# syzhang092218-source/dgppo

Measured on AMD Instinct MI355X. Metric: env-steps/sec whole node, LidarSpread n=8 4096 envs, 1/2/4/8 GPUs, higher is better.
Workload: dtype f32

## Files before the change

### dgppo_amd/csrc/nn_graph.hip

```cpp
#include "common.h"

struct Topo {
  int n, ng, gs, os, per, lidar, spread;
  int S, Ns;
};

static Topo make_topo(const dgppo_env_cfg& c) {
  Topo t;
  t.n = c.n_agents; t.ng = c.n_goals; t.gs = cfg_goal_slots(c); t.os = cfg_obs_slots(c);
  t.lidar = cfg_is_lidar(c) ? 1 : 0; t.spread = cfg_is_spread(c) ? 1 : 0;
  t.per = t.os;
  t.S = t.n + t.gs + t.os;
  t.Ns = t.n + t.ng + cfg_obs_nodes(c);
  return t;
}

__device__ inline int sender_node(const Topo& t, int i, int s) {
  if (s < t.n) return s;
  if (s < t.n + t.gs) return t.spread ? t.n + (s - t.n) : t.n + i;
  const int m = s - t.n - t.gs;
  return t.lidar ? t.n + t.ng + i * t.per + m : t.n + t.ng + m;
}
__device__ inline int slot_of(const Topo& t, int nd, int i) {
  if (nd < t.n) return nd;
// ... 165 lines not shown
  const float* qt;
  const float* Xa;
  const float* Xo;
  const float* efeat;
  const float* emask;
  float* zcat;
  float* attn;
  const float* dzcat;
  float* dqt;
  float* dXa;
  float* dXo;
  int relu_xo;
  int G;
  const float* Xo_raw; const float* Wo; const float* bo; int ldwo;
  float* dwo_slab;
};

__global__ void __launch_bounds__(256) attn_fwd_valu_kernel(AttnArgs a) {
  extern __shared__ float sm[];
  const Topo& t = a.t;
  const int g = blockIdx.x, tid = threadIdx.x, nt = blockDim.x;
  const int n = t.n, S = t.S, Ns = t.Ns, F = a.F, H = a.H, Fl = F + 1;
  float* s_x = sm;
  float* s_q = s_x + Ns * Fl;
  float* s_e = s_q + n * H * Fl;
  float* s_m = s_e + n * S * 4;
  float* s_a = s_m + n * S;
  for (int idx = tid; idx < Ns * F; idx += nt) {
    const int nd = idx / F, f = idx - nd * F;
    s_x[nd * Fl + f] = (nd < n) ? a.Xa[((size_t)g * n + nd) * F + f] : a.Xo[((size_t)g * (Ns - n) + (nd - n)) * F + f];
// ... 354 lines not shown
  return __int_as_float(__builtin_amdgcn_update_dpp(0, __float_as_int(v), CTRL, 0xf, 0xf, false));
}
__device__ inline float grp8_sum(float v) {
  v += dpp_f<0xB1>(v);
  v += dpp_f<0x4E>(v);
  v += dpp_f<0x141>(v);
  return v;
}
__device__ inline float grp8_max(float v) {
  v = fmaxf(v, dpp_f<0xB1>(v));
  v = fmaxf(v, dpp_f<0x4E>(v));
  v = fmaxf(v, dpp_f<0x141>(v));
  return v;
}

template <int H, int NPA, int SJ>
__global__ void __launch_bounds__(256) attn_fwd_slot8_kernel(AttnArgs a) {
  constexpr int F = 8, Wd = F + 4;
  const Topo& t = a.t;
  const int lane = threadIdx.x & 63, wave = threadIdx.x >> 6, sub = lane & 7, grp = lane >> 3;
  const int g = __builtin_amdgcn_readfirstlane(blockIdx.x * 4 + wave);
  if (g >= a.G) return;
  const int n = t.n, S = t.S, Ns = t.Ns, Kp = a.Kp, kc = F + H * Wd;
  const float* Xa = a.Xa + (size_t)g * n * F;
  const float* Xo = a.Xo + (size_t)g * (Ns - n) * F - (size_t)n * F;
  const float* qt = a.qt + (size_t)g * n * H * F;
  const float* ef = a.efeat + (size_t)g * n * S * 4;
  const float* mk = a.emask + (size_t)g * n * S;
  float* zc = a.zcat + (size_t)g * n * Kp;
  float* at = a.attn + (size_t)g * n * S * H;
  for (int idx = lane; idx < n * 2; idx += 64)
    *reinterpret_cast<float4*>(zc + (idx >> 1) * Kp + 4 * (idx & 1)) = reinterpret_cast<const float4*>(Xa)[idx];
  for (int i = lane; i < n; i += 64)
    for (int c = kc; c < Kp; ++c) zc[i * Kp + c] = (c == kc) ? ones_col(a.t, mk + i * S) : 0.0f;
#pragma unroll
  for (int p = 0; p < NPA; ++p) {
    const int ia = grp + 8 * p;
    const bool live = ia < n;
    const int i = live ? ia : n - 1;
    float4 q[H][2], x[SJ][2], e[SJ];
    float m[SJ];
#pragma unroll
    for (int h = 0; h < H; ++h) {
      const float4* qp = reinterpret_cast<const float4*>(qt + (i * H + h) * F);
      q[h][0] = qp[0]; q[h][1] = qp[1];
    }
#pragma unroll
    for (int j = 0; j < SJ; ++j) {
      int sl = sub + 8 * j;
      sl = sl < S ? sl : S - 1;
      const int nd = sender_node(t, i, sl);
      const float4* xp = reinterpret_cast<const float4*>((nd < n ? Xa : Xo) + (size_t)nd * F);
      x[j][0] = xp[0]; x[j][1] = xp[1];
      e[j] = reinterpret_cast<const float4*>(ef)[i * S + sl];
      m[j] = mk[i * S + sl];
    }
    float av[SJ][H];
#pragma unroll
    for (int h = 0; h < H; ++h) {
      float mx = -INFINITY;
#pragma unroll
      for (int j = 0; j < SJ; ++j) {
        const bool ok = live && (sub + 8 * j) < S && m[j] != 0.0f;
        float acc = q[h][0].x * x[j][0].x;
        acc = fmaf(q[h][0].y, x[j][0].y, acc); acc = fmaf(q[h][0].z, x[j][0].z, acc); acc = fmaf(q[h][0].w, x[j][0].w, acc);
        acc = fmaf(q[h][1].x, x[j][1].x, acc); acc = fmaf(q[h][1].y, x[j][1].y, acc);
        acc = fmaf(q[h][1].z, x[j][1].z, acc); acc = fmaf(q[h][1].w, x[j][1].w, acc);
        av[j][h] = ok ? acc : -INFINITY;
        mx = fmaxf(mx, av[j][h]);
      }
      mx = grp8_max(mx);
      float den = 0.0f;
#pragma unroll
      for (int j = 0; j < SJ; ++j) {
        const float ev = (av[j][h] == -INFINITY) ? 0.0f : __expf(av[j][h] - mx);
        av[j][h] = ev;
        den += ev;
      }
      den = grp8_sum(den);
      const float inv = (den > 0.0f) ? 1.0f / den : 0.0f;
#pragma unroll
      for (int j = 0; j < SJ; ++j) av[j][h] *= inv;
    }
#pragma unroll
    for (int j = 0; j < SJ; ++j) {
      const int sl = sub + 8 * j;
      if (live && sl < S) {
#pragma unroll
        for (int h = 0; h < H; ++h) if (a.attn != nullptr) at[(i * S + sl) * H + h] = av[j][h];
      }
    }
#pragma unroll
    for (int h = 0; h < H; ++h) {
      float z[Wd];
#pragma unroll
      for (int c = 0; c < Wd; ++c) z[c] = 0.0f;
#pragma unroll
      for (int j = 0; j < SJ; ++j) {
        const float w = av[j][h];
        if (w != 0.0f) {
          z[0] = fmaf(w, x[j][0].x, z[0]); z[1] = fmaf(w, x[j][0].y, z[1]); z[2] = fmaf(w, x[j][0].z, z[2]); z[3] = fmaf(w, x[j][0].w, z[3]);
          z[4] = fmaf(w, x[j][1].x, z[4]); z[5] = fmaf(w, x[j][1].y, z[5]); z[6] = fmaf(w, x[j][1].z, z[6]); z[7] = fmaf(w, x[j][1].w, z[7]);
          z[8] = fmaf(w, e[j].x, z[8]); z[9] = fmaf(w, e[j].y, z[9]); z[10] = fmaf(w, e[j].z, z[10]); z[11] = fmaf(w, e[j].w, z[11]);
        }
      }
#pragma unroll
      for (int c = 0; c < Wd; ++c) z[c] = grp8_sum(z[c]);
      if (live && sub == h) {
        float4* o = reinterpret_cast<float4*>(zc + i * Kp + F + h * Wd);
        o[0] = make_float4(z[0], z[1], z[2], z[3]);
        o[1] = make_float4(z[4], z[5], z[6], z[7]);
        o[2] = make_float4(z[8], z[9], z[10], z[11]);
      }
    }
  }
}

template <int H, int NPA, int SJ>
__global__ void __launch_bounds__(256) attn_bwd_slot8_kernel(AttnArgs a) {
  constexpr int F = 8, Wd = F + 4;
  const Topo& t = a.t;
  const int lane = threadIdx.x & 63, wave = threadIdx.x >> 6, sub = lane & 7, grp = lane >> 3;
  const int g = __builtin_amdgcn_readfirstlane(blockIdx.x * 4 + wave);
  if (g >= a.G) return;
  const int n = t.n, S = t.S, Ns = t.Ns, Kp = a.Kp;
  const float* Xa = a.Xa + (size_t)g * n * F;
  const float* Xo = a.Xo + (size_t)g * (Ns - n) * F - (size_t)n * F;
// ... 57 lines not shown
          o[0] = fmaf(dl, x[j][0].x, o[0]); o[1] = fmaf(dl, x[j][0].y, o[1]); o[2] = fmaf(dl, x[j][0].z, o[2]); o[3] = fmaf(dl, x[j][0].w, o[3]);
          o[4] = fmaf(dl, x[j][1].x, o[4]); o[5] = fmaf(dl, x[j][1].y, o[5]); o[6] = fmaf(dl, x[j][1].z, o[6]); o[7] = fmaf(dl, x[j][1].w, o[7]);
        }
      }
#pragma unroll
      for (int c = 0; c < F; ++c) o[c] = grp8_sum(o[c]);
      if (live && sub == h) {
        float4* op = reinterpret_cast<float4*>(dq + (i * H + h) * F);
        op[0] = make_float4(o[0], o[1], o[2], o[3]);
        op[1] = make_float4(o[4], o[5], o[6], o[7]);
      }
    }
  }
}

template <int H, int NPA>
static bool launch_attn_slot8_sj(const AttnArgs& a, int SJ, int grid, hipStream_t s, bool bwd) {
#define DGPPO_SJ(J)                                                                                              \
  case J:                                                                                                        \
    if (bwd) hipLaunchKernelGGL((attn_bwd_slot8_kernel<H, NPA, J>), dim3(grid), dim3(256), 0, s, a);             \
    else hipLaunchKernelGGL((attn_fwd_slot8_kernel<H, NPA, J>), dim3(grid), dim3(256), 0, s, a);                 \
    return true;
  switch (SJ) {
    DGPPO_SJ(1) DGPPO_SJ(2) DGPPO_SJ(3) DGPPO_SJ(4) DGPPO_SJ(5) DGPPO_SJ(6) DGPPO_SJ(7) DGPPO_SJ(8)
    default: return false;
  }
#undef DGPPO_SJ
}
static bool attn_slot8_shape(const Topo& t, int F, int H) { return F == 8 && H == 3 && t.n <= 32 && t.S <= 64; }
static bool launch_attn_slot8(const AttnArgs& a, hipStream_t s, bool bwd) {
  if (!attn_slot8_shape(a.t, a.F, a.H)) return false;
  const int grid = (a.G + 3) / 4, NPA = (a.t.n + 7) / 8, SJ = (a.t.S + 7) / 8;
  switch (NPA) {
    case 1: return launch_attn_slot8_sj<3, 1>(a, SJ, grid, s, bwd);
    case 2: return launch_attn_slot8_sj<3, 2>(a, SJ, grid, s, bwd);
    case 3: return launch_attn_slot8_sj<3, 3>(a, SJ, grid, s, bwd);
    case 4: return launch_attn_slot8_sj<3, 4>(a, SJ, grid, s, bwd);
    default: return false;
  }
}

#define ABD_XL 36
#define ABD_DZL 40
typedef float4 abd_f4;
__device__ inline f32x4g mfma4(float a_, float b_, f32x4g c_) { return __builtin_amdgcn_mfma_f32_4x4x1f32(a_, b_, c_, 0, 0, 0); }
__device__ inline const float* f4e(const float4& v) { return reinterpret_cast<const float*>(&v); }
__device__ inline float4 ld4_if(bool ok, const float4* p) {
  float4 v = make_float4(0.f, 0.f, 0.f, 0.f);
  if (ok) v = *p;
  return v;
}

// ... 1112 lines not shown
                                  float* attn, int32_t G, void* stream) {
  AttnArgs a{};
  int32_t rc = attn_check(cfg, F, H, Kp, G, a);
  if (rc) return rc;
  if (G == 0) return 0;
  DGPPO_REQUIRE(qt && Xa && efeat && emask && zcat, "attn_fwd: NULL operand");
  DGPPO_REQUIRE(a.t.Ns == a.t.n || Xo, "attn_fwd: Xo is NULL");
  a.qt = qt; a.Xa = Xa; a.Xo = Xo; a.efeat = efeat; a.emask = emask; a.zcat = zcat; a.attn = attn;
  const Topo& t = a.t;
  const hipStream_t s = (hipStream_t)stream;
  const size_t smem = sizeof(float) * ((size_t)t.Ns * (F + 1) + (size_t)t.n * H * (F + 1) + (size_t)t.n * t.S * 5 +
                                       (size_t)t.n * t.S * H);
  DGPPO_REQUIRE(smem <= 64 * 1024, "attn_fwd: graph too large for LDS (%zu B)", smem);
  bool launched = true;
  switch (attn_family(t, F, H, Kp, false, false)) {
    case AttnFamily::SLOT8: launched = launch_attn_slot8(a, s, false); break;
    case AttnFamily::BD: launched = launch_attn_bd(a, s, false); break;
    case AttnFamily::MFMA:
      hipLaunchKernelGGL(attn_fwd_kernel, dim3(G), dim3(256), attn_mfma_smem(attn_dims(t, F, H), false), s, a);
      break;
    case AttnFamily::VALU: hipLaunchKernelGGL(attn_fwd_valu_kernel, dim3(G), dim3(256), smem, s, a); break;
  }
  DGPPO_REQUIRE(launched, "attn_fwd: dispatch failed");
  DGPPO_LAUNCH_CHECK();
  return 0;
}

extern "C" int32_t dgppo_attn_bwd(const dgppo_env_cfg* cfg, int32_t F, int32_t H, int32_t Kp, const float* dzcat,
                                  const float* attn, const float* qt, const float* Xa, const float* Xo,
                                  const float* efeat, float* dqt, float* dXa, float* dXo, int32_t relu_xo, int32_t G,
                                  void* stream) {
  AttnArgs a{};
  int32_t rc = attn_check(cfg, F, H, Kp, G, a);
  if (rc) return rc;
  if (G == 0) return 0;
  DGPPO_REQUIRE(dzcat && attn && qt && Xa && efeat && dqt, "attn_bwd: NULL operand");
  DGPPO_REQUIRE(a.t.Ns == a.t.n || Xo, "attn_bwd: Xo is NULL");
  DGPPO_REQUIRE(!(dXo && !dXa), "attn_bwd: dXo needs dXa");
  a.dzcat = dzcat; a.attn = (float*)attn; a.qt = qt; a.Xa = Xa; a.Xo = Xo; a.efeat = efeat; a.dqt = dqt; a.dXa = dXa; a.dXo = dXo;
  const Topo& t = a.t;
  const hipStream_t s = (hipStream_t)stream;
  const size_t smem = sizeof(float) * ((size_t)t.Ns * (F + 1) + (size_t)t.n * H * (F + 1) + (size_t)t.n * t.S * 4 +
                                       2 * (size_t)t.n * t.S * H + (size_t)t.n * H * (F + 5));
  DGPPO_REQUIRE(smem <= 64 * 1024, "attn_bwd: graph too large for LDS (%zu B)", smem);
  const AttnFamily fam = attn_family(t, F, H, Kp, true, dXa != nullptr);
  a.relu_xo = (relu_xo && dXo && fam == AttnFamily::BD) ? 1 : 0;
  bool launched = true;
  switch (fam) {
    case AttnFamily::SLOT8: launched = launch_attn_slot8(a, s, true); break;
    case AttnFamily::BD: launched = launch_attn_bd(a, s, true); break;
    case AttnFamily::MFMA:
      hipLaunchKernelGGL(attn_bwd_kernel, dim3(G), dim3(256), attn_mfma_smem(attn_dims(t, F, H), true), s, a);
      break;
    case AttnFamily::VALU: hipLaunchKernelGGL(attn_bwd_valu_kernel, dim3(G), dim3(256), smem, s, a); break;
  }
  DGPPO_REQUIRE(launched, "attn_bwd: dispatch failed");
  DGPPO_LAUNCH_CHECK();
  if (relu_xo && dXo && !a.relu_xo)
    return dgppo_relu_bwd(dXo, Xo, (int64_t)G * (t.Ns - t.n) * F, stream);
  return 0;
}

static bool attn_xo_ok(const Topo& t, int F, int H, int Kp) {
  return t.Ns > t.n && attn_family(t, F, H, Kp, true, true) == AttnFamily::BD;
}
extern "C" int32_t dgppo_attn_xo_supported(const dgppo_env_cfg* cfg, int32_t F, int32_t H, int32_t Kp) {
  AttnArgs a{};
  if (attn_check(cfg, F, H, Kp, 0, a)) return 0;
  return attn_xo_ok(a.t, F, H, Kp) ? 1 : 0;
}
extern "C" int32_t dgppo_attn_fwd_xo(const dgppo_env_cfg* cfg, int32_t F, int32_t H, int32_t Kp, const float* qt, const float* Xa,
                                     const float* Xo_raw, const float* Wo, int32_t ldwo, const float* bo, const float* efeat,
                                     const float* emask, float* zcat, float* attn, int32_t G, void* stream) {
  AttnArgs a{};
// ... 79 lines not shown
```

### dgppo_amd/nets.py

```python
from __future__ import annotations

import math
from typing import Dict, List, Optional, Tuple

import numpy as np
import torch

from . import _native as N
from . import ops_nn as K

H_HEADS = 3
MSG_DIM = 32
OUT_DIM = 64
HID = 64


def _ceil4(x):
    return (x + 3) // 4 * 4


class Layout:
    def __init__(self):
        self.entries: Dict[str, Tuple[int, Tuple[int, ...]]] = {}
        self.size = 0
# ... 162 lines not shown
        for l, (f, fp, d, kp) in enumerate(self.dims):
            q = lambda nm: self.p(f"gnn{l}.{nm}")
            K.gnn_prep(q("Wq"), q("bq"), q("Wk"), q("Wv"), q("bv"), q("We"), q("Wu"), self.pp(f"gnn{l}.Mcat"),
                       self.pp(f"gnn{l}.cvec"), self.pp(f"gnn{l}.Wout"), f, fp, d, H_HEADS, kp)

    def _xo_fusable(self, l: int) -> bool:
        if l != 0 or self.gnn_layers != 2:
            return False
        key = "_xo_ok"
        if not hasattr(self, key):
            f1, fp1, d1, kp1 = self.dims[1]
            setattr(self, key, self.dims[0][1] == 8 and self.dims[0][2] == 32 and fp1 == 32 and
                    K.attn_xo_supported(self.cfg, fp1, H_HEADS, kp1))
        return getattr(self, key)

    def zero_grads(self):
        self.grads.zero_()

    def forward(self, feats: GraphFeats, n_seq: int, T: int, h0: Optional[torch.Tensor], tag: str = "f",
                hs_out: Optional[torch.Tensor] = None, train: bool = True):
        cfg, G, A = self.cfg, feats.G, self.arena
        n = cfg.n_agents
        R = G * n
        Ro = G * feats.n_other
        act = {"feats": feats, "G": G, "n_seq": n_seq, "T": T}
        Xa, Xo = feats.Xa, feats.Xo
        xo_fused = None
        for l, (f, fp, d, kp) in enumerate(self.dims):
            qt = A.get(f"{tag}.qt{l}", R, H_HEADS * fp)
            K.dense_fwd(Xa, self.pp(f"gnn{l}.Mcat"), self.pp(f"gnn{l}.cvec"), qt)
            zcat = A.get(f"{tag}.zcat{l}", R, kp)
            attn = A.get(f"{tag}.attn{l}", R, cfg.fan_in, H_HEADS) if train else None
            if xo_fused is not None:
                K.attn_fwd_xo(cfg, fp, H_HEADS, kp, qt, Xa, xo_fused[0], xo_fused[1], xo_fused[2], feats.efeat, feats.emask, zcat, attn, G)
            else:
                K.attn_fwd(cfg, fp, H_HEADS, kp, qt, Xa, Xo if Ro > 0 else None, feats.efeat, feats.emask, zcat, attn, G)
            act[f"xo_fused{l}"] = xo_fused
            xo_fused = None
            Xa_n = A.get(f"{tag}.Xa{l + 1}", R, d)
            K.dense_fwd(zcat, self.pp(f"gnn{l}.Wout"), self.p(f"gnn{l}.bu"), Xa_n, act=1)
            act[f"Xa{l}"], act[f"Xo{l}"], act[f"qt{l}"], act[f"zcat{l}"], act[f"attn{l}"] = Xa, Xo, qt, zcat, attn
            if l < self.gnn_layers - 1 and Ro > 0:
                if self._xo_fusable(l):
                    xo_fused = (Xo, self.pp(f"gnn{l}.Wout")[:fp], self.p(f"gnn{l}.bu"))
                    Xo = None
                else:
                    Xo_n = A.get(f"{tag}.Xo{l + 1}", Ro, d)
                    K.dense_fwd(Xo, self.pp(f"gnn{l}.Wout")[:fp], self.p(f"gnn{l}.bu"), Xo_n, act=1)
                    Xo = Xo_n
            Xa = Xa_n
        act[f"Xa{self.gnn_layers}"] = Xa
        if self.kind == "Vl":
            pooled = A.get(f"{tag}.pool", G, OUT_DIM)
            K.mean_agents(Xa, pooled, G, n, OUT_DIM)
            x, Rh, n_inner = pooled, G, 1
# ... 343 lines not shown
```

### dgppo_amd/ops_nn.py

```python
from __future__ import annotations

import ctypes as C
from typing import Optional

import torch

from . import _native as N

FLOPS = [0.0]


def _mat(t: torch.Tensor, name: str):
    if t.dim() != 2:
        raise ValueError(f"{name} must be 2-D, got {tuple(t.shape)}")
    if not t.is_cuda:
        raise RuntimeError(f"{name} must live on the GPU (the HIP path has no CPU fallback)")
    if t.dtype != torch.float32:
        raise TypeError(f"{name} must be float32")
    if t.shape[1] > 1 and t.stride(1) != 1:
        raise ValueError(f"{name} must have unit inner stride")
    ld = t.stride(0) if t.shape[0] > 1 else max(t.shape[1], t.stride(0))
    return C.c_void_p(t.data_ptr()), int(ld), int(t.shape[0]), int(t.shape[1])


# ... 240 lines not shown
    N.check(rc, "dgppo_attn_fwd")


def attn_bwd(cfg, F, H, Kp, dzcat, attn, qt, Xa, Xo, efeat, dqt, dXa, dXo, G, relu_xo: bool = False):
    n = cfg.n_agents
    N.expect_shape(dzcat, (G * n, Kp), "dzcat")
    N.expect_shape(dqt, (G * n, H * F), "dqt")
    if dXa is not None:
        N.expect_shape(dXa, (G * n, F), "dXa")
    FLOPS[0] += 4.0 * G * n * H * cfg.fan_in * (2 * F + 4)
    rc = N.lib().dgppo_attn_bwd(C.byref(cfg), F, H, Kp, _p(dzcat), _p(attn), _p(qt), _p(Xa), _p(Xo), _p(efeat), _p(dqt),
                                _p(dXa), _p(dXo), int(relu_xo), G, N.stream_ptr())
    N.check(rc, "dgppo_attn_bwd")


def attn_xo_supported(cfg, F, H, Kp) -> bool:
    return bool(N.lib().dgppo_attn_xo_supported(C.byref(cfg), F, H, Kp))


def _wo_ptr(Wo):
    if not Wo.is_cuda or Wo.dtype != torch.float32:
        raise TypeError("Wo must be a float32 GPU tensor")
    return C.c_void_p(Wo.data_ptr())


def _wo_ld(Wo):
    if Wo.dim() != 2 or Wo.shape[0] != 8 or Wo.shape[1] < 32 or Wo.stride(1) != 1:
        raise ValueError(f"Wo must be [8, >= 32] with contiguous rows, got {tuple(Wo.shape)} strides {Wo.stride()}")
    return int(Wo.stride(0))

# ... 143 lines not shown
```

### include/dgppo_hip.h

```cpp
#ifndef DGPPO_HIP_H
#define DGPPO_HIP_H

#include <stdint.h>

#ifdef __cplusplus
extern "C" {
#endif

#define DGPPO_ABI_VERSION 3

enum {
  DGPPO_ENV_LIDAR_SPREAD = 0,
  DGPPO_ENV_LIDAR_TARGET = 1,
  DGPPO_ENV_LIDAR_BICYCLE_TARGET = 2,
  DGPPO_ENV_MPE_SPREAD = 3,
  DGPPO_ENV_MPE_TARGET = 4,
  DGPPO_ENV_LIDAR_LINE = 5,
  DGPPO_ENV_MPE_LINE = 6,
  DGPPO_ENV_MPE_FORMATION = 7,
  DGPPO_ENV_MPE_CORRIDOR = 8,
  DGPPO_ENV_MPE_CONNECT_SPREAD = 9,
  DGPPO_ENV_VMAS_REVERSE_TRANSPORT = 10
};
enum {
// ... 119 lines not shown
                            const float* b1, const float* W2, const float* b2, float* hs, float* hprev, float* gates,
                            float* u, float* out, int32_t M, int32_t n_out, void* stream);
int64_t dgppo_dense_bwd_w_workspace_bytes(int32_t K, int32_t N);

int32_t dgppo_graph_feats(const dgppo_env_cfg* cfg, const float* agent, int64_t agent_se, int64_t agent_st,
                          const float* goal, const float* obst, const float* hits, int64_t hits_se, int64_t hits_st,
                          const int32_t* env_ids, int32_t n_env, int32_t n_time, float* Xa, float* Xo, float* efeat,
                          float* emask, int32_t Fp, void* stream);

int32_t dgppo_attn_fwd(const dgppo_env_cfg* cfg, int32_t F, int32_t H, int32_t Kp, const float* qt, const float* Xa,
                       const float* Xo, const float* efeat, const float* emask, float* zcat, float* attn, int32_t G,
                       void* stream);
int32_t dgppo_attn_bwd(const dgppo_env_cfg* cfg, int32_t F, int32_t H, int32_t Kp, const float* dzcat,
                       const float* attn, const float* qt, const float* Xa, const float* Xo, const float* efeat,
                       float* dqt, float* dXa, float* dXo, int32_t relu_xo, int32_t G, void* stream);
int32_t dgppo_attn_xo_supported(const dgppo_env_cfg* cfg, int32_t F, int32_t H, int32_t Kp);
int32_t dgppo_attn_fwd_xo(const dgppo_env_cfg* cfg, int32_t F, int32_t H, int32_t Kp, const float* qt, const float* Xa,
                          const float* Xo_raw, const float* Wo, int32_t ldwo, const float* bo, const float* efeat,
                          const float* emask, float* zcat, float* attn, int32_t G, void* stream);
int32_t dgppo_attn_bwd_xo(const dgppo_env_cfg* cfg, int32_t F, int32_t H, int32_t Kp, const float* dzcat,
                          const float* attn, const float* qt, const float* Xa, const float* Xo_raw, const float* Wo,
                          int32_t ldwo, const float* bo, const float* efeat, float* dqt, float* dXa, float* dXo,
                          int32_t relu_xo, int32_t G, void* stream);
int64_t dgppo_attn_xo_workspace_bytes(int32_t G);
int32_t dgppo_attn_bwd_xo_dw(const dgppo_env_cfg* cfg, int32_t F, int32_t H, int32_t Kp, const float* dzcat,
                             const float* attn, const float* qt, const float* Xa, const float* Xo_raw, const float* Wo,
                             int32_t ldwo, const float* bo, const float* efeat, float* dqt, float* dXa, float* dWo,
                             int32_t lddwo, float* dbo, float* workspace, int64_t workspace_bytes, int32_t G, void* stream);

int32_t dgppo_gnn_prep(const float* Wq, const float* bq, const float* Wk, const float* Wv, const float* bv,
// ... 66 lines not shown
```

Baseline: 4.085 million.

## Fuse GNN layer-0 query projection, attention, output dense and next-layer query

Adds a fused first-layer GNN forward kernel. It computes the query projection with MFMA inside the slot8 attention kernel, runs attention, then applies the Wout dense with ReLU from LDS-staged weights and optionally the next layer's query projection. The kernel loops persistently over graphs, one wave per graph. This removes three separate dense launches and the global round trips of qt0, zcat and qt1 inputs, and skips writing zcat outside training. In exchange it uses more LDS and registers, adds shape restrictions (H=3, D0 32 or 64), and creates a second forward path that must match the unfused one numerically.

```diff
diff --git a/dgppo_amd/csrc/nn_graph.hip b/dgppo_amd/csrc/nn_graph.hip
--- a/dgppo_amd/csrc/nn_graph.hip
+++ b/dgppo_amd/csrc/nn_graph.hip
@@ -203,6 +203,9 @@
   int G;
   const float* Xo_raw; const float* Wo; const float* bo; int ldwo;
   float* dwo_slab;
+  const float* Mcat0; const float* cvec0; const float* Wout0; const float* bu0; int ldwout;
+  const float* Mcat1; const float* cvec1;
+  float* Xa1; float* qt1;
 };
 
 __global__ void __launch_bounds__(256) attn_fwd_valu_kernel(AttnArgs a) {
@@ -587,103 +590,280 @@
   return v;
 }
 
-template <int H, int NPA, int SJ>
-__global__ void __launch_bounds__(256) attn_fwd_slot8_kernel(AttnArgs a) {
+__device__ inline void wave_lds_fence() {
+  __builtin_amdgcn_fence(__ATOMIC_ACQ_REL, "wavefront");
+  __builtin_amdgcn_wave_barrier();
+}
+template <int NPA, int D0, bool NEXT> struct Slot8Lds {
+  static constexpr int MT = (NPA + 1) / 2, ROWS = 16 * MT;
+  static constexpr int NW = D0 == 0 ? 4 : (MT == 1 ? 8 : 4);
+  static constexpr int TL = D0 + 4 > 52 ? D0 + 4 : 52, QL = 28;
+  static constexpr int WB0 = 12 * D0 + 16, W0 = 4 * WB0;
+  static constexpr int WB1 = 8 * 96 + 16, W1 = NEXT ? 4 * WB1 : 0;
+  static constexpr int NB = D0 + (NEXT ? 96 : 0);
+  static constexpr int WAVE = ROWS * (TL + QL);
+  static constexpr int TOTAL = D0 == 0 ? 4 : W0 + W1 + NB + NW * WAVE;
+  static constexpr int NV0 = 48 * D0 / 4, NV1 = NEXT ? 32 * 96 / 4 : 0;
+  static constexpr int NST = D0 == 0 ? 1 : (NV0 + NV1 + NW * 64 - 1) / (NW * 64);
+};
+template <int H, int NPA, int SJ, int D0, bool NEXT>
+__global__ void __launch_bounds__((Slot8Lds<NPA, D0, NEXT>::NW * 64)) attn_fwd_slot8_kernel(AttnArgs a) {
   constexpr int F = 8, Wd = F + 4;
+  constexpr bool FUSED = D0 != 0;
+  using L = Slot8Lds<NPA, D0, NEXT>;
+  constexpr int NW = L::NW, TL = L::TL;
+  static_assert(!FUSED || (H == 3 && (D0 == 32 || D0 == 64) && (!NEXT || D0 == 32)), "fused first layer: H = 3, D0 = 32 (+ next) or 64");
+  __shared__ float4 s8_sm[(L::TOTAL + 3) / 4];
   const Topo& t = a.t;
-  const int lane = threadIdx.x & 63, wave = threadIdx.x >> 6, sub = lane & 7, grp = lane >> 3;
-  const int g = __builtin_amdgcn_readfirstlane(blockIdx.x * 4 + wave);
-  if (g >= a.G) return;
+  const int lane0 = threadIdx.x & 63, wave = threadIdx.x >> 6;
   const int n = t.n, S = t.S, Ns = t.Ns, Kp = a.Kp, kc = F + H * Wd;
-  const float* Xa = a.Xa + (size_t)g * n * F;
-  const float* Xo = a.Xo + (size_t)g * (Ns - n) * F - (size_t)n * F;
-  const float* qt = a.qt + (size_t)g * n * H * F;
-  const float* ef = a.efeat + (size_t)g * n * S * 4;
-  const float* mk = a.emask + (size_t)g * n * S;
-  float* zc = a.zcat + (size_t)g * n * Kp;
-  float* at = a.attn + (size_t)g * n * S * H;
-  for (int idx = lane; idx < n * 2; idx += 64)
-    *reinterpret_cast<float4*>(zc + (idx >> 1) * Kp + 4 * (idx & 1)) = reinterpret_cast<const float4*>(Xa)[idx];
-  for (int i = lane; i < n; i += 64)
-    for (int c = kc; c < Kp; ++c) zc[i * Kp + c] = (c == kc) ? ones_col(a.t, mk + i * S) : 0.0f;
-#pragma unroll
-  for (int p = 0; p < NPA; ++p) {
-    const int ia = grp + 8 * p;
-    const bool live = ia < n;
-    const int i = live ? ia : n - 1;
-    float4 q[H][2], x[SJ][2], e[SJ];
-    float m[SJ];
-#pragma unroll
-    for (int h = 0; h < H; ++h) {
-      const float4* qp = reinterpret_cast<const float4*>(qt + (i * H + h) * F);
-      q[h][0] = qp[0]; q[h][1] = qp[1];
-    }
-#pragma unroll
-    for (int j = 0; j < SJ; ++j) {
-      int sl = sub + 8 * j;
-      sl = sl < S ? sl : S - 1;
-      const int nd = sender_node(t, i, sl);
-      const float4* xp = reinterpret_cast<const float4*>((nd < n ? Xa : Xo) + (size_t)nd * F);
-      x[j][0] = xp[0]; x[j][1] = xp[1];
-      e[j] = reinterpret_cast<const float4*>(ef)[i * S + sl];
-      m[j] = mk[i * S + sl];
-    }
-    float av[SJ][H];
-#pragma unroll
-    for (int h = 0; h < H; ++h) {
-      float mx = -INFINITY;
-#pragma unroll
-      for (int j = 0; j < SJ; ++j) {
-        const bool ok = live && (sub + 8 * j) < S && m[j] != 0.0f;
-        float acc = q[h][0].x * x[j][0].x;
-        acc = fmaf(q[h][0].y, x[j][0].y, acc); acc = fmaf(q[h][0].z, x[j][0].z, acc); acc = fmaf(q[h][0].w, x[j][0].w, acc);
-        acc = fmaf(q[h][1].x, x[j][1].x, acc); acc = fmaf(q[h][1].y, x[j][1].y, acc);
-        acc = fmaf(q[h][1].z, x[j][1].z, acc); acc = fmaf(q[h][1].w, x[j][1].w, acc);
-        av[j][h] = ok ? acc : -INFINITY;
-        mx = fmaxf(mx, av[j][h]);
-      }
-      mx = grp8_max(mx);
-      float den = 0.0f;
-#pragma unroll
-      for (int j = 0; j < SJ; ++j) {
-        const float ev = (av[j][h] == -INFINITY) ? 0.0f : __expf(av[j][h] - mx);
-        av[j][h] = ev;
-        den += ev;
-      }
-      den = grp8_sum(den);
-      const float inv = (den > 0.0f) ? 1.0f / den : 0.0f;
-#pragma unroll
-      for (int j = 0; j < SJ; ++j) av[j][h] *= inv;
-    }
-#pragma unroll
-    for (int j = 0; j < SJ; ++j) {
-      const int sl = sub + 8 * j;
-      if (live && sl < S) {
-#pragma unroll
-        for (int h = 0; h < H; ++h) if (a.attn != nullptr) at[(i * S + sl) * H + h] = av[j][h];
-      }
-    }
-#pragma unroll
-    for (int h = 0; h < H; ++h) {
-      float z[Wd];
-#pragma unroll
-      for (int c = 0; c < Wd; ++c) z[c] = 0.0f;
-#pragma unroll
-      for (int j = 0; j < SJ; ++j) {
-        const float w = av[j][h];
-        if (w != 0.0f) {
-          z[0] = fmaf(w, x[j][0].x, z[0]); z[1] = fmaf(w, x[j][0].y, z[1]); z[2] = fmaf(w, x[j][0].z, z[2]); z[3] = fmaf(w, x[j][0].w, z[3]);
-          z[4] = fmaf(w, x[j][1].x, z[4]); z[5] = fmaf(w, x[j][1].y, z[5]); z[6] = fmaf(w, x[j][1].z, z[6]); z[7] = fmaf(w, x[j][1].w, z[7]);
-          z[8] = fmaf(w, e[j].x, z[8]); z[9] = fmaf(w, e[j].y, z[9]); z[10] = fmaf(w, e[j].z, z[10]); z[11] = fmaf(w, e[j].w, z[11]);
-        }
-      }
-#pragma unroll
-      for (int c = 0; c < Wd; ++c) z[c] = grp8_sum(z[c]);
-      if (live && sub == h) {
-        float4* o = reinterpret_cast<float4*>(zc + i * Kp + F + h * Wd);
-        o[0] = make_float4(z[0], z[1], z[2], z[3]);
-        o[1] = make_float4(z[4], z[5], z[6], z[7]);
-        o[2] = make_float4(z[8], z[9], z[10], z[11]);
+  float* W0s = reinterpret_cast<float*>(s8_sm);
+  float* W1s = W0s + L::W0;
+  float* Bs = W1s + L::W1;
+  float* zt = Bs + L::NB + wave * L::WAVE;
+  float* qs = zt + L::ROWS * TL;
+  float4 stage[L::NST];
+  float bstage = 0.0f, m0[2][2], cv0[2];
+  if constexpr (FUSED) {
+#pragma unroll
+    for (int j = 0; j < L::NST; ++j) {
+      const int idx = threadIdx.x + j * NW * 64;
+      stage[j] = make_float4(0.f, 0.f, 0.f, 0.f);
+      if (idx < L::NV0) stage[j] = *reinterpret_cast<const float4*>(a.Wout0 + (size_t)(idx / (D0 / 4)) * a.ldwout + 4 * (idx % (D0 / 4)));
+      else if (idx < L::NV0 + L::NV1) stage[j] = reinterpret_cast<const float4*>(a.Mcat1)[idx - L::NV0];
+    }
+    if ((int)threadIdx.x < D0) bstage = a.bu0[threadIdx.x];
+    else if (NEXT && (int)threadIdx.x < L::NB) bstage = a.cvec1[threadIdx.x - D0];
+#pragma unroll
+    for (int ct = 0; ct < 2; ++ct) {
+      const int li = lane0 & 15, lq = lane0 >> 4;
+      const int col = ct * 16 + li, cc = col < H * F ? col : 0;
+      cv0[ct] = col < H * F ? a.cvec0[cc] : 0.0f;
+#pragma unroll
+      for (int s2 = 0; s2 < 2; ++s2) m0[s2][ct] = col < H * F ? a.Mcat0[(2 * lq + s2) * H * F + cc] : 0.0f;
+    }
+  }
+  const int iters = FUSED ? (a.G + gridDim.x * NW - 1) / (gridDim.x * NW) : 1;
+  for (int it = 0; it < iters; ++it) {
+    const int g = __builtin_amdgcn_readfirstlane((it * gridDim.x + blockIdx.x) * NW + wave);
+    const bool active = g < a.G;
+    int lane = lane0;
+    if constexpr (FUSED) asm volatile("" : "+v"(lane));
+    const int sub = lane & 7, grp = lane >> 3, li = lane & 15, lq = lane >> 4;
+    if (active) {
+      const float* Xa = a.Xa + (size_t)g * n * F;
+      const float* Xo = a.Xo + (size_t)g * (Ns - n) * F - (size_t)n * F;
+      const float* qt = a.qt + (size_t)g * n * H * F;
+      const float* ef = a.efeat + (size_t)g * n * S * 4;
+      const float* mk = a.emask + (size_t)g * n * S;
+      float* zc = a.zcat + (size_t)g * n * Kp;
+      float* at = a.attn + (size_t)g * n * S * H;
+      const bool keep_z = !FUSED || a.zcat != nullptr;
+      if (keep_z) {
+        for (int idx = lane; idx < n * 2; idx += 64)
+          *reinterpret_cast<float4*>(zc + (idx >> 1) * Kp + 4 * (idx & 1)) = reinterpret_cast<const float4*>(Xa)[idx];
+        for (int i = lane; i < n; i += 64)
+          for (int c = kc; c < Kp; ++c) zc[i * Kp + c] = (c == kc) ? ones_col(a.t, mk + i * S) : 0.0f;
+      }
+#pragma unroll
+      for (int p = 0; p < NPA; ++p) {
+        const int ia = grp + 8 * p;
+        const bool live = ia < n;
+        const int i = live ? ia : n - 1;
+        float4 q[H][2], x[SJ][2], e[SJ];
+        float m[SJ];
+        float4 xi0, xi1;
+        if constexpr (FUSED) {
+          xi0 = reinterpret_cast<const float4*>(Xa + i * F)[0];
+          xi1 = reinterpret_cast<const float4*>(Xa + i * F)[1];
+        } else {
+#pragma unroll
+          for (int h = 0; h < H; ++h) {
+            const float4* qp = reinterpret_cast<const float4*>(qt + (i * H + h) * F);
+            q[h][0] = qp[0]; q[h][1] = qp[1];
+          }
+        }
+#pragma unroll
+        for (int j = 0; j < SJ; ++j) {
+          int sl = sub + 8 * j;
+          sl = sl < S ? sl : S - 1;
+          const int nd = sender_node(t, i, sl);
+          const float4* xp = reinterpret_cast<const float4*>((nd < n ? Xa : Xo) + (size_t)nd * F);
+          x[j][0] = xp[0]; x[j][1] = xp[1];
+          e[j] = reinterpret_cast<const float4*>(ef)[i * S + sl];
+          m[j] = mk[i * S + sl];
+        }
+        if constexpr (FUSED) {
+          if ((p & 1) == 0) {
+            const int r0 = 8 * p, ra = r0 + li < n ? r0 + li : n - 1;
+            const float2 xk = *reinterpret_cast<const float2*>(Xa + ra * F + 2 * lq);
+#pragma unroll
+            for (int ct = 0; ct < 2; ++ct) {
+              f32x4g acc = {cv0[ct], cv0[ct], cv0[ct], cv0[ct]};
+              acc = __builtin_amdgcn_mfma_f32_16x16x4f32(xk.x, m0[0][ct], acc, 0, 0, 0);
+              acc = __builtin_amdgcn_mfma_f32_16x16x4f32(xk.y, m0[1][ct], acc, 0, 0, 0);
+              if (ct * 16 + li < H * F) {
+#pragma unroll
+                for (int r = 0; r < 4; ++r) qs[(r0 + 4 * lq + r) * L::QL + ct * 16 + li] = acc[r];
+              }
+            }
+            wave_lds_fence();
+          }
+#pragma unroll
+          for (int h = 0; h < H; ++h) {
+            q[h][0] = *reinterpret_cast<const float4*>(qs + ia * L::QL + h * F);
+            q[h][1] = *reinterpret_cast<const float4*>(qs + ia * L::QL + h * F + 4);
+          }
+          if (live && sub == 3) {
+            *reinterpret_cast<float4*>(zt + ia * TL) = xi0;
+            *reinterpret_cast<float4*>(zt + ia * TL + 4) = xi1;
+          }
+          float one = 1.0f;
+          if (t.gs == 0) {
+            float any = 0.0f;
+#pragma unroll
+            for (int j = 0; j < SJ; ++j) any = m[j] != 0.0f ? 1.0f : any;
+            one = grp8_max(any);
+          }
+          if (live && sub == 4) *reinterpret_cast<float4*>(zt + ia * TL + kc) = make_float4(one, 0.f, 0.f, 0.f);
+        }
+        float av[SJ][H];
+#pragma unroll
+        for (int h = 0; h < H; ++h) {
+          float mx = -INFINITY;
+#pragma unroll
+          for (int j = 0; j < SJ; ++j) {
+            const bool ok = live && (sub + 8 * j) < S && m[j] != 0.0f;
+            float acc = q[h][0].x * x[j][0].x;
+            acc = fmaf(q[h][0].y, x[j][0].y, acc); acc = fmaf(q[h][0].z, x[j][0].z, acc); acc = fmaf(q[h][0].w, x[j][0].w, acc);
+            acc = fmaf(q[h][1].x, x[j][1].x, acc); acc = fmaf(q[h][1].y, x[j][1].y, acc);
+            acc = fmaf(q[h][1].z, x[j][1].z, acc); acc = fmaf(q[h][1].w, x[j][1].w, acc);
+            av[j][h] = ok ? acc : -INFINITY;
+            mx = fmaxf(mx, av[j][h]);
+          }
+          mx = grp8_max(mx);
+          float den = 0.0f;
+#pragma unroll
+          for (int j = 0; j < SJ; ++j) {
+            const float ev = (av[j][h] == -INFINITY) ? 0.0f : __expf(av[j][h] - mx);
+            av[j][h] = ev;
+            den += ev;
+          }
+          den = grp8_sum(den);
+          const float inv = (den > 0.0f) ? 1.0f / den : 0.0f;
+#pragma unroll
+          for (int j = 0; j < SJ; ++j) av[j][h] *= inv;
+        }
+#pragma unroll
+        for (int j = 0; j < SJ; ++j) {
+          const int sl = sub + 8 * j;
+          if (live && sl < S) {
+#pragma unroll
+            for (int h = 0; h < H; ++h) if (a.attn != nullptr) at[(i * S + sl) * H + h] = av[j][h];
+          }
+        }
+#pragma unroll
+        for (int h = 0; h < H; ++h) {
+          float z[Wd];
+#pragma unroll
+          for (int c = 0; c < Wd; ++c) z[c] = 0.0f;
+#pragma unroll
+          for (int j = 0; j < SJ; ++j) {
+            const float w = av[j][h];
+            if (w != 0.0f) {
+              z[0] = fmaf(w, x[j][0].x, z[0]); z[1] = fmaf(w, x[j][0].y, z[1]); z[2] = fmaf(w, x[j][0].z, z[2]); z[3] = fmaf(w, x[j][0].w, z[3]);
+              z[4] = fmaf(w, x[j][1].x, z[4]); z[5] = fmaf(w, x[j][1].y, z[5]); z[6] = fmaf(w, x[j][1].z, z[6]); z[7] = fmaf(w, x[j][1].w, z[7]);
+              z[8] = fmaf(w, e[j].x, z[8]); z[9] = fmaf(w, e[j].y, z[9]); z[10] = fmaf(w, e[j].z, z[10]); z[11] = fmaf(w, e[j].w, z[11]);
+            }
+          }
+#pragma unroll
+          for (int c = 0; c < Wd; ++c) z[c] = grp8_sum(z[c]);
+          if (live && sub == h) {
+            if (keep_z) {
+              float4* o = reinterpret_cast<float4*>(zc + i * Kp + F + h * Wd);
+              o[0] = make_float4(z[0], z[1], z[2], z[3]);
+              o[1] = make_float4(z[4], z[5], z[6], z[7]);
+              o[2] = make_float4(z[8], z[9], z[10], z[11]);
+            }
+            if constexpr (FUSED) {
+              float4* o = reinterpret_cast<float4*>(zt + ia * TL + F + h * Wd);
+              o[0] = make_float4(z[0], z[1], z[2], z[3]);
+              o[1] = make_float4(z[4], z[5], z[6], z[7]);
+              o[2] = make_float4(z[8], z[9], z[10], z[11]);
+            }
+          }
+        }
+      }
+    }
+    if constexpr (FUSED) {
+      if (it == 0) {
+#pragma unroll
+        for (int j = 0; j < L::NST; ++j) {
+          const int idx = threadIdx.x + j * NW * 64;
+          if (idx < L::NV0) {
+            const int k = idx / (D0 / 4), c4 = idx % (D0 / 4);
+            *reinterpret_cast<float4*>(W0s + (k / 12) * L::WB0 + (k % 12) * D0 + 4 * c4) = stage[j];
+          } else if (idx < L::NV0 + L::NV1) {
+            const int k = (idx - L::NV0) / 24, c4 = (idx - L::NV0) % 24;
+            *reinterpret_cast<float4*>(W1s + (k / 8) * L::WB1 + (k % 8) * 96 + 4 * c4) = stage[j];
+          }
+        }
+        if ((int)threadIdx.x < L::NB) Bs[threadIdx.x] = bstage;
+        __syncthreads();
+      }
+      if (active) {
+        wave_lds_fence();
+#pragma unroll
+        for (int mt = 0; mt < L::MT; ++mt) {
+          const int r0 = mt * 16;
+          float za[12];
+#pragma unroll
+          for (int c = 0; c < 3; ++c) {
+            const float4 v = *reinterpret_cast<const float4*>(zt + (r0 + li) * TL + lq * 12 + 4 * c);
+            za[4 * c] = v.x; za[4 * c + 1] = v.y; za[4 * c + 2] = v.z; za[4 * c + 3] = v.w;
+          }
+          wave_lds_fence();
+#pragma unroll 1
+          for (int ct = 0; ct < D0 / 16; ++ct) {
+            const float b = Bs[ct * 16 + li];
+            f32x4g acc = {b, b, b, b};
+#pragma unroll
+            for (int s = 0; s < 12; ++s)
+              acc = __builtin_amdgcn_mfma_f32_16x16x4f32(za[s], W0s[lq * L::WB0 + s * D0 + ct * 16 + li], acc, 0, 0, 0);
+#pragma unroll
+            for (int r = 0; r < 4; ++r) zt[(r0 + 4 * lq + r) * TL + ct * 16 + li] = fmaxf(acc[r], 0.0f);
+          }
+          wave_lds_fence();
+          float* Xa1 = a.Xa1 + (size_t)g * n * D0;
+#pragma unroll
+          for (int j = 0; j < 16 * D0 / 4 / 64; ++j) {
+            const int idx = lane + 64 * j, row = r0 + idx / (D0 / 4), c4 = idx % (D0 / 4);
+            if (row < n) *reinterpret_cast<float4*>(Xa1 + row * D0 + 4 * c4) = *reinterpret_cast<const float4*>(zt + row * TL + 4 * c4);
+          }
+          if constexpr (NEXT) {
+            float xa[8];
+#pragma unroll
+            for (int c = 0; c < 2; ++c) {
+              const float4 v = *reinterpret_cast<const float4*>(zt + (r0 + li) * TL + lq * 8 + 4 * c);
+              xa[4 * c] = v.x; xa[4 * c + 1] = v.y; xa[4 * c + 2] = v.z; xa[4 * c + 3] = v.w;
+            }
+            float* qt1 = a.qt1 + (size_t)g * n * 96;
+#pragma unroll 1
+            for (int ct = 0; ct < 6; ++ct) {
+              const float b = Bs[D0 + ct * 16 + li];
+              f32x4g acc = {b, b, b, b};
+#pragma unroll
+              for (int s = 0; s < 8; ++s)
+                acc = __builtin_amdgcn_mfma_f32_16x16x4f32(xa[s], W1s[lq * L::WB1 + s * 96 + ct * 16 + li], acc, 0, 0, 0);
+#pragma unroll
+              for (int r = 0; r < 4; ++r) {
+                const int row = r0 + 4 * lq + r;
+                if (row < n) qt1[row * 96 + ct * 16 + li] = acc[r];
+              }
+            }
+          }
+        }
+        wave_lds_fence();
       }
     }
   }
@@ -771,12 +951,35 @@
   }
 }
 
-template <int H, int NPA>
-static bool launch_attn_slot8_sj(const AttnArgs& a, int SJ, int grid, hipStream_t s, bool bwd) {
-#define DGPPO_SJ(J)                                                                                              \
-  case J:                                                                                                        \
-    if (bwd) hipLaunchKernelGGL((attn_bwd_slot8_kernel<H, NPA, J>), dim3(grid), dim3(256), 0, s, a);             \
-    else hipLaunchKernelGGL((attn_fwd_slot8_kernel<H, NPA, J>), dim3(grid), dim3(256), 0, s, a);                 \
+template <int H, int NPA, int SJ, int D0, bool NEXT>
+static int slot8_fused_grid(int G) {
+  constexpr int NW = Slot8Lds<NPA, D0, NEXT>::NW;
+  static thread_local int cap = 0, cap_dev = -1;
+  int dev = 0;
+  if (hipGetDevice(&dev) != hipSuccess) dev = 0;
+  if (cap == 0 || dev != cap_dev) {
+    int per_cu = 0, cus = 256;
+    if (hipOccupancyMaxActiveBlocksPerMultiprocessor(&per_cu, reinterpret_cast<const void*>(&attn_fwd_slot8_kernel<H, NPA, SJ, D0, NEXT>),
+                                                     NW * 64, 0) != hipSuccess || per_cu < 1) per_cu = 1;
+    if (hipDeviceGetAttribute(&cus, hipDeviceAttributeMultiprocessorCount, dev) != hipSuccess || cus < 1) cus = 256;
+    cap = per_cu * cus;
+    cap_dev = dev;
+  }
+  const int blocks = (G + NW - 1) / NW;
+  return blocks < cap ? blocks : cap;
+}
+template <int H, int NPA, int D0, bool NEXT>
+static bool launch_attn_slot8_sj(const AttnArgs& a, int SJ, hipStream_t s, bool bwd) {
+#define DGPPO_SJ(J)                                                                                                        \
+  case J:                                                                                                                  \
+    if constexpr (D0 == 0) {                                                                                               \
+      const int grid = (a.G + 3) / 4;                                                                                      \
+      if (bwd) hipLaunchKernelGGL((attn_bwd_slot8_kernel<H, NPA, J>), dim3(grid), dim3(256), 0, s, a);                     \
+      else hipLaunchKernelGGL((attn_fwd_slot8_kernel<H, NPA, J, 0, false>), dim3(grid), dim3(256), 0, s, a);               \
+    } else {                                                                                                               \
+      hipLaunchKernelGGL((attn_fwd_slot8_kernel<H, NPA, J, D0, NEXT>), dim3(slot8_fused_grid<H, NPA, J, D0, NEXT>(a.G)),   \
+                         dim3(Slot8Lds<NPA, D0, NEXT>::NW * 64), 0, s, a);                                                 \
+    }                                                                                                                      \
     return true;
   switch (SJ) {
     DGPPO_SJ(1) DGPPO_SJ(2) DGPPO_SJ(3) DGPPO_SJ(4) DGPPO_SJ(5) DGPPO_SJ(6) DGPPO_SJ(7) DGPPO_SJ(8)
@@ -785,14 +988,15 @@
 #undef DGPPO_SJ
 }
 static bool attn_slot8_shape(const Topo& t, int F, int H) { return F == 8 && H == 3 && t.n <= 32 && t.S <= 64; }
+template <int D0, bool NEXT>
 static bool launch_attn_slot8(const AttnArgs& a, hipStream_t s, bool bwd) {
   if (!attn_slot8_shape(a.t, a.F, a.H)) return false;
-  const int grid = (a.G + 3) / 4, NPA = (a.t.n + 7) / 8, SJ = (a.t.S + 7) / 8;
+  const int NPA = (a.t.n + 7) / 8, SJ = (a.t.S + 7) / 8;
   switch (NPA) {
-    case 1: return launch_attn_slot8_sj<3, 1>(a, SJ, grid, s, bwd);
-    case 2: return launch_attn_slot8_sj<3, 2>(a, SJ, grid, s, bwd);
-    case 3: return launch_attn_slot8_sj<3, 3>(a, SJ, grid, s, bwd);
-    case 4: return launch_attn_slot8_sj<3, 4>(a, SJ, grid, s, bwd);
+    case 1: return launch_attn_slot8_sj<3, 1, D0, NEXT>(a, SJ, s, bwd);
+    case 2: return launch_attn_slot8_sj<3, 2, D0, NEXT>(a, SJ, s, bwd);
+    case 3: return launch_attn_slot8_sj<3, 3, D0, NEXT>(a, SJ, s, bwd);
+    case 4: return launch_attn_slot8_sj<3, 4, D0, NEXT>(a, SJ, s, bwd);
     default: return false;
   }
 }
@@ -1935,7 +2139,7 @@
   DGPPO_REQUIRE(smem <= 64 * 1024, "attn_fwd: graph too large for LDS (%zu B)", smem);
   bool launched = true;
   switch (attn_family(t, F, H, Kp, false, false)) {
-    case AttnFamily::SLOT8: launched = launch_attn_slot8(a, s, false); break;
+    case AttnFamily::SLOT8: launched = launch_attn_slot8<0, false>(a, s, false); break;
     case AttnFamily::BD: launched = launch_attn_bd(a, s, false); break;
     case AttnFamily::MFMA:
       hipLaunchKernelGGL(attn_fwd_kernel, dim3(G), dim3(256), attn_mfma_smem(attn_dims(t, F, H), false), s, a);
@@ -1955,9 +2159,10 @@
   int32_t rc = attn_check(cfg, F, H, Kp, G, a);
   if (rc) return rc;
   if (G == 0) return 0;
-  DGPPO_REQUIRE(dzcat && attn && qt && Xa && efeat && dqt, "attn_bwd: NULL operand");
+  DGPPO_REQUIRE(dzcat && attn && Xa && efeat && dqt, "attn_bwd: NULL operand");
   DGPPO_REQUIRE(a.t.Ns == a.t.n || Xo, "attn_bwd: Xo is NULL");
   DGPPO_REQUIRE(!(dXo && !dXa), "attn_bwd: dXo needs dXa");
+  DGPPO_REQUIRE(qt || attn_family(a.t, F, H, Kp, true, dXa != nullptr) == AttnFamily::SLOT8, "attn_bwd: qt is NULL");
   a.dzcat = dzcat; a.attn = (float*)attn; a.qt = qt; a.Xa = Xa; a.Xo = Xo; a.efeat = efeat; a.dqt = dqt; a.dXa = dXa; a.dXo = dXo;
   const Topo& t = a.t;
   const hipStream_t s = (hipStream_t)stream;
@@ -1968,7 +2173,7 @@
   a.relu_xo = (relu_xo && dXo && fam == AttnFamily::BD) ? 1 : 0;
   bool launched = true;
   switch (fam) {
-    case AttnFamily::SLOT8: launched = launch_attn_slot8(a, s, true); break;
+    case AttnFamily::SLOT8: launched = launch_attn_slot8<0, false>(a, s, true); break;
     case AttnFamily::BD: launched = launch_attn_bd(a, s, true); break;
     case AttnFamily::MFMA:
       hipLaunchKernelGGL(attn_bwd_kernel, dim3(G), dim3(256), attn_mfma_smem(attn_dims(t, F, H), true), s, a);
@@ -1979,6 +2184,45 @@
   DGPPO_LAUNCH_CHECK();
   if (relu_xo && dXo && !a.relu_xo)
     return dgppo_relu_bwd(dXo, Xo, (int64_t)G * (t.Ns - t.n) * F, stream);
+  return 0;
+}
+
+static bool gnn_layer0_ok(const Topo& t, int Kp, int D0, bool has_next) {
+  return Kp == 48 && attn_slot8_shape(t, 8, 3) && ((D0 == 32 && has_next) || (D0 == 64 && !has_next));
+}
+extern "C" int32_t dgppo_gnn_layer0_supported(const dgppo_env_cfg* cfg, int32_t Kp, int32_t D0, int32_t has_next) {
+  AttnArgs a{};
+  if (attn_check(cfg, 8, 3, Kp, 0, a)) return 0;
+  return gnn_layer0_ok(a.t, Kp, D0, has_next != 0) ? 1 : 0;
+}
+extern "C" int32_t dgppo_gnn_layer0_fwd(const dgppo_env_cfg* cfg, int32_t Kp, int32_t D0, const float* Xa, const float* Xo,
+                                        const float* efeat, const float* emask, const float* Mcat0, const float* cvec0,
+                                        const float* Wout0, int32_t ldwout, const float* bu0, const float* Mcat1,
+                                        const float* cvec1, float* Xa1, float* qt1, float* zcat, float* attn, int32_t G,
+                                        void* stream) {
+  AttnArgs a{};
+  int32_t rc = attn_check(cfg, 8, 3, Kp, G, a);
+  if (rc) return rc;
+  const bool has_next = Mcat1 != nullptr;
+  DGPPO_REQUIRE(gnn_layer0_ok(a.t, Kp, D0, has_next),
+                "gnn_layer0_fwd: no fused kernel for this shape (Kp=%d D0=%d next=%d n=%d S=%d; ask dgppo_gnn_layer0_supported)", Kp, D0,
+                (int)has_next, a.t.n, a.t.S);
+  if (G == 0) return 0;
+  DGPPO_REQUIRE(Xa && efeat && emask && Mcat0 && cvec0 && Wout0 && bu0 && Xa1, "gnn_layer0_fwd: NULL operand");
+  DGPPO_REQUIRE(a.t.Ns == a.t.n || Xo, "gnn_layer0_fwd: Xo is NULL");
+  DGPPO_REQUIRE(!has_next || (cvec1 && qt1), "gnn_layer0_fwd: Mcat1 needs cvec1 and qt1");
+  DGPPO_REQUIRE(has_next || (!cvec1 && !qt1), "gnn_layer0_fwd: cvec1 / qt1 without Mcat1");
+  DGPPO_REQUIRE(ldwout >= D0 && (ldwout & 3) == 0, "gnn_layer0_fwd: ldwout=%d must be a multiple of 4, >= D0=%d", ldwout, D0);
+  DGPPO_REQUIRE(((reinterpret_cast<uintptr_t>(Wout0) | reinterpret_cast<uintptr_t>(Mcat1) | reinterpret_cast<uintptr_t>(Xa1) |
+                  reinterpret_cast<uintptr_t>(Xa) | reinterpret_cast<uintptr_t>(efeat) | reinterpret_cast<uintptr_t>(zcat)) & 15) == 0,
+                "gnn_layer0_fwd: Xa, efeat, Wout0, Mcat1, Xa1 and zcat must be 16-byte aligned");
+  a.Xa = Xa; a.Xo = Xo; a.efeat = efeat; a.emask = emask; a.zcat = zcat; a.attn = attn;
+  a.Mcat0 = Mcat0; a.cvec0 = cvec0; a.Wout0 = Wout0; a.ldwout = ldwout; a.bu0 = bu0; a.Mcat1 = Mcat1; a.cvec1 = cvec1;
+  a.Xa1 = Xa1; a.qt1 = qt1;
+  const bool launched = has_next ? launch_attn_slot8<32, true>(a, (hipStream_t)stream, false)
+                                 : launch_attn_slot8<64, false>(a, (hipStream_t)stream, false);
+  DGPPO_REQUIRE(launched, "gnn_layer0_fwd: dispatch failed");
+  DGPPO_LAUNCH_CHECK();
   return 0;
 }
 
diff --git a/dgppo_amd/nets.py b/dgppo_amd/nets.py
--- a/dgppo_amd/nets.py
+++ b/dgppo_amd/nets.py
@@ -200,6 +200,13 @@
                     K.attn_xo_supported(self.cfg, fp1, H_HEADS, kp1))
         return getattr(self, key)
 
+    def _layer0_fused(self) -> bool:
+        key = "_l0_ok"
+        if not hasattr(self, key):
+            f, fp, d, kp = self.dims[0]
+            setattr(self, key, fp == 8 and K.gnn_layer0_supported(self.cfg, kp, d, self.gnn_layers > 1))
+        return getattr(self, key)
+
     def zero_grads(self):
         self.grads.zero_()
 
@@ -212,19 +219,31 @@
         act = {"feats": feats, "G": G, "n_seq": n_seq, "T": T}
         Xa, Xo = feats.Xa, feats.Xo
         xo_fused = None
+        qt_next = None
         for l, (f, fp, d, kp) in enumerate(self.dims):
-            qt = A.get(f"{tag}.qt{l}", R, H_HEADS * fp)
-            K.dense_fwd(Xa, self.pp(f"gnn{l}.Mcat"), self.pp(f"gnn{l}.cvec"), qt)
-            zcat = A.get(f"{tag}.zcat{l}", R, kp)
+            Xa_n = A.get(f"{tag}.Xa{l + 1}", R, d)
             attn = A.get(f"{tag}.attn{l}", R, cfg.fan_in, H_HEADS) if train else None
-            if xo_fused is not None:
-                K.attn_fwd_xo(cfg, fp, H_HEADS, kp, qt, Xa, xo_fused[0], xo_fused[1], xo_fused[2], feats.efeat, feats.emask, zcat, attn, G)
+            if l == 0 and self._layer0_fused():
+                nxt = self.gnn_layers > 1
+                qt, zcat = None, (A.get(f"{tag}.zcat{l}", R, kp) if train else None)
+                qt_next = A.get(f"{tag}.qt{l + 1}", R, H_HEADS * d) if nxt else None
+                K.gnn_layer0_fwd(cfg, kp, Xa, Xo if Ro > 0 else None, feats.efeat, feats.emask, self.pp("gnn0.Mcat"),
+                                 self.pp("gnn0.cvec"), self.pp("gnn0.Wout"), self.p("gnn0.bu"),
+                                 self.pp("gnn1.Mcat") if nxt else None, self.pp("gnn1.cvec") if nxt else None, Xa_n, qt_next,
+                                 zcat, attn, G)
             else:
-                K.attn_fwd(cfg, fp, H_HEADS, kp, qt, Xa, Xo if Ro > 0 else None, feats.efeat, feats.emask, zcat, attn, G)
+                qt, qt_next = qt_next, None
+                if qt is None:
+                    qt = A.get(f"{tag}.qt{l}", R, H_HEADS * fp)
+                    K.dense_fwd(Xa, self.pp(f"gnn{l}.Mcat"), self.pp(f"gnn{l}.cvec"), qt)
+                zcat = A.get(f"{tag}.zcat{l}", R, kp)
+                if xo_fused is not None:
+                    K.attn_fwd_xo(cfg, fp, H_HEADS, kp, qt, Xa, xo_fused[0], xo_fused[1], xo_fused[2], feats.efeat, feats.emask, zcat, attn, G)
+                else:
+                    K.attn_fwd(cfg, fp, H_HEADS, kp, qt, Xa, Xo if Ro > 0 else None, feats.efeat, feats.emask, zcat, attn, G)
+                K.dense_fwd(zcat, self.pp(f"gnn{l}.Wout"), self.p(f"gnn{l}.bu"), Xa_n, act=1)
             act[f"xo_fused{l}"] = xo_fused
             xo_fused = None
-            Xa_n = A.get(f"{tag}.Xa{l + 1}", R, d)
-            K.dense_fwd(zcat, self.pp(f"gnn{l}.Wout"), self.p(f"gnn{l}.bu"), Xa_n, act=1)
             act[f"Xa{l}"], act[f"Xo{l}"], act[f"qt{l}"], act[f"zcat{l}"], act[f"attn{l}"] = Xa, Xo, qt, zcat, attn
             if l < self.gnn_layers - 1 and Ro > 0:
                 if self._xo_fusable(l):
diff --git a/dgppo_amd/ops_nn.py b/dgppo_amd/ops_nn.py
--- a/dgppo_amd/ops_nn.py
+++ b/dgppo_amd/ops_nn.py
@@ -278,6 +278,44 @@
     N.check(rc, "dgppo_attn_bwd")
 
 
+def gnn_layer0_supported(cfg, Kp: int, D0: int, has_next: bool) -> bool:
+    return bool(N.lib().dgppo_gnn_layer0_supported(C.byref(cfg), int(Kp), int(D0), int(has_next)))
+
+
+def gnn_layer0_fwd(cfg, Kp, Xa, Xo, efeat, emask, Mcat0, cvec0, Wout0, bu0, Mcat1, cvec1, Xa1, qt1, zcat, attn, G):
+    n, S, F, H = cfg.n_agents, cfg.fan_in, 8, 3
+    R = G * n
+    D0 = int(Xa1.shape[1])
+    N.expect_shape(Xa, (R, F), "Xa")
+    if cfg.num_nodes - 1 - n > 0:
+        N.expect_shape(Xo, (G * (cfg.num_nodes - 1 - n), F), "Xo")
+    N.expect_shape(efeat, (R, S, 4), "efeat")
+    N.expect_shape(emask, (R, S), "emask")
+    N.expect_shape(Mcat0, (F, H * F), "Mcat0")
+    N.expect_shape(cvec0, (H * F,), "cvec0")
+    wp, ldw, wr, wc = _mat(Wout0, "Wout0")
+    if (wr, wc) != (Kp, D0):
+        raise ValueError(f"gnn_layer0_fwd: Wout0 must be [{Kp}, {D0}], got {tuple(Wout0.shape)}")
+    N.expect_shape(bu0, (D0,), "bu0")
+    N.expect_shape(Xa1, (R, D0), "Xa1")
+    if (Mcat1 is None) != (qt1 is None) or (Mcat1 is None) != (cvec1 is None):
+        raise ValueError("gnn_layer0_fwd: Mcat1, cvec1 and qt1 go together")
+    if Mcat1 is not None:
+        N.expect_shape(Mcat1, (D0, 3 * D0), "Mcat1")
+        N.expect_shape(cvec1, (3 * D0,), "cvec1")
+        N.expect_shape(qt1, (R, 3 * D0), "qt1")
+    if zcat is not None:
+        N.expect_shape(zcat, (R, Kp), "zcat")
+    if attn is not None:
+        N.expect_shape(attn, (R, S, H), "attn")
+    FLOPS[0] += 2.0 * R * F * H * F + 2.0 * G * n * H * S * (2 * F + 4) + 2.0 * R * Kp * D0
+    if Mcat1 is not None:
+        FLOPS[0] += 2.0 * R * D0 * 3 * D0
+    rc = N.lib().dgppo_gnn_layer0_fwd(C.byref(cfg), int(Kp), D0, _p(Xa), _p(Xo), _p(efeat), _p(emask), _p(Mcat0), _p(cvec0), wp, ldw,
+                                      _p(bu0), _p(Mcat1), _p(cvec1), _p(Xa1), _p(qt1), _p(zcat), _p(attn), G, N.stream_ptr())
+    N.check(rc, "dgppo_gnn_layer0_fwd")
+
+
 def attn_xo_supported(cfg, F, H, Kp) -> bool:
     return bool(N.lib().dgppo_attn_xo_supported(C.byref(cfg), F, H, Kp))
 
diff --git a/include/dgppo_hip.h b/include/dgppo_hip.h
--- a/include/dgppo_hip.h
+++ b/include/dgppo_hip.h
@@ -157,6 +157,11 @@
 int32_t dgppo_attn_bwd(const dgppo_env_cfg* cfg, int32_t F, int32_t H, int32_t Kp, const float* dzcat,
                        const float* attn, const float* qt, const float* Xa, const float* Xo, const float* efeat,
                        float* dqt, float* dXa, float* dXo, int32_t relu_xo, int32_t G, void* stream);
+int32_t dgppo_gnn_layer0_supported(const dgppo_env_cfg* cfg, int32_t Kp, int32_t D0, int32_t has_next);
+int32_t dgppo_gnn_layer0_fwd(const dgppo_env_cfg* cfg, int32_t Kp, int32_t D0, const float* Xa, const float* Xo,
+                             const float* efeat, const float* emask, const float* Mcat0, const float* cvec0,
+                             const float* Wout0, int32_t ldwout, const float* bu0, const float* Mcat1, const float* cvec1,
+                             float* Xa1, float* qt1, float* zcat, float* attn, int32_t G, void* stream);
 int32_t dgppo_attn_xo_supported(const dgppo_env_cfg* cfg, int32_t F, int32_t H, int32_t Kp);
 int32_t dgppo_attn_fwd_xo(const dgppo_env_cfg* cfg, int32_t F, int32_t H, int32_t Kp, const float* qt, const float* Xa,
                           const float* Xo_raw, const float* Wo, int32_t ldwo, const float* bo, const float* efeat,
```

After: 4.146 million, median of 6. +1.5%, better.
